# GuoYi0/alphaFive

Measured on AMD Instinct MI355X. Metric: self-play moves/sec (11x11, 500 sims/move), higher is better.
Workload: dtype f32 (fp16x2 split operands: 3 fp16 MFMA products per MAC, fp32 accumulate)

## Files before the change

alphafive_amd/csrc/af_engine.hip:

```cpp

#include <hip/hip_runtime.h>
#include <stdint.h>
#include <stdio.h>
#include <stdlib.h>
#include <string.h>

#include <type_traits>
#include <vector>

#include "af_engine.h"
#include "af_noise.h"

typedef unsigned long long u64;

enum { PH_IDLE = 0, PH_MOVE_START = 1, PH_SEARCH = 2, PH_MOVE_DONE = 3, PH_ERROR = 4, PH_DESCENT = 5  };
enum { CT_SIMS = 0, CT_SELECTS, CT_EXPANDS, CT_TERMINALS, CT_PLIES, CT_EPISODES, CT_LSUM, CT_LEXP,
       CT_GC, CT_GC_SCANNED, CT_YIELDS, CT_STALLS, CT_N };
enum { HIST_WORK = 0, HIST_TIME = 64, HIST_MAXTIME = 96, HIST_N = 97 };

struct EngineParams {
    int G, S, C, goal, sims, upper, training, mode, node_cap, max_ply, budget, budget_hard;
    uint32_t hash_mask;
    double init_temp, tau_decay, tau_decay_r, alpha, c_puct;
    float c_puct32;
// ... 191 lines not shown
            if (dir == 3) run_mask<KW, true>(theirs, d, P.goal, valid, wt);
            else run_mask<KW, false>(theirs, d, P.goal, valid, wt);
        } else if (dir == 3) {
            run_mask<KW, true>(mine, d, P.goal, valid, wm);
            run_mask<KW, true>(theirs, d, P.goal, valid, wt);
        } else {
            run_mask<KW, false>(mine, d, P.goal, valid, wm);
            run_mask<KW, false>(theirs, d, P.goal, valid, wt);
        }
#pragma unroll
        for (int k = 0; k < KW; ++k) any[k] = wm[k] | wt[k];
        const int f = bb_first<KW>(any);
        if (f >= 0) {
            const int key = f * 4 + dir;
            if (key < best_key) { best_key = key; best_v = bb_test<KW>(wm, f) ? 1.0f : -1.0f; }
        }
    }
    if (best_key != 0x7fffffff) { *value = best_v; return 1; }
    bool full = true;
#pragma unroll
    for (int k = 0; k < KW; ++k) full = full && ((mine[k] | theirs[k]) == P.boardmask[k]);
    *value = 0.0f;
    return full ? 1 : 0;
}

template <int KW>
__device__ __forceinline__ int terminal_through_last(const EngineParams& P, const u64* mine, const u64* theirs, int last, uint32_t inv_s16,
                                                     int lane, float* value) {
    const int S = P.S, g1 = P.goal - 1;
    const int y0 = (int)(((uint32_t)last * inv_s16) >> 16), x0 = last - y0 * S;
    const int dir = lane >> 4, j = (lane & 15) - g1;
    const int dy = dir == 1 ? 0 : (dir == 3 ? -1 : 1), dx = dir == 0 ? 0 : 1;
    const int y = y0 + j * dy, x = x0 + j * dx;
    const bool inb = (lane & 15) <= 2 * g1 && (unsigned)y < (unsigned)S && (unsigned)x < (unsigned)S;
    const int c = inb ? y * S + x : 0;
    u64 word = theirs[0];
#pragma unroll
    for (int k = 1; k < KW; ++k) word = (c >> 6) == k ? theirs[k] : word;
    const u64 w = __ballot(inb && ((word >> (c & 63)) & 1ull));
    u64 r = w;
    for (int t = 1; t <= g1; ++t) r &= w >> t;
    if (r) { *value = -1.0f; return 1; }
    bool full = true;
#pragma unroll
    for (int k = 0; k < KW; ++k) full = full && ((mine[k] | theirs[k]) == P.boardmask[k]);
    *value = 0.0f;
    return full ? 1 : 0;
}

template <int KW>
__host__ __device__ __forceinline__ uint32_t key_hash(const u64* mine, const u64* theirs) {
    u64 h = 0x9E3779B97F4A7C15ull;
#pragma unroll
    for (int k = 0; k < KW; ++k) {
        h = (h ^ mine[k]) * 0xff51afd7ed558ccdull;
        h ^= h >> 29;
        h = (h ^ theirs[k]) * 0xc4ceb9fe1a85ec53ull;
        h ^= h >> 32;
    }
    return (uint32_t)h;
}

template <int KW>
__device__ int tree_lookup(const EngineParams& P, int g, const u64* mine, const u64* theirs, int lane, uint32_t* slot_out) {
    const uint32_t* slots = P.hash + (size_t)g * (P.hash_mask + 1);
    const u64* keys = P.node_key + (size_t)g * P.node_cap * (2 * KW);
    const uint32_t h = key_hash<KW>(mine, theirs);
    for (uint32_t round = 0; round <= P.hash_mask / 64 + 1; ++round) {
        const uint32_t s = (h + round * 64 + lane) & P.hash_mask;
        const uint32_t v = slots[s];
        const u64 empties = __ballot(v == 0);
        const int first_empty = empties ? __builtin_ctzll(empties) : 64;
        bool match = false;
        if (v != 0 && lane < first_empty) {
            const u64* kk = keys + (size_t)(v - 1) * (2 * KW);
            match = true;
#pragma unroll
            for (int k = 0; k < KW; ++k) match = match && kk[k] == mine[k] && kk[KW + k] == theirs[k];
        }
        const u64 mm = __ballot(match);
        if (mm) {
            const int src = __builtin_ctzll(mm);
            return __builtin_amdgcn_readlane((int)v, src) - 1;
        }
        if (first_empty < 64) {
            *slot_out = (h + round * 64 + first_empty) & P.hash_mask;
            return -1;
        }
    }
    *slot_out = 0xffffffffu;
    return -1;
}

template <int KW>
__device__ __forceinline__ uint32_t memo_bucket(const EngineParams& P, const u64* mine, const u64* theirs, int last) {
    uint32_t h = key_hash<KW>(mine, theirs) ^ ((uint32_t)(last + 1) * 0x9E3779B1u);
    h ^= h >> 15; h *= 0x85EBCA6Bu; h ^= h >> 13;
    return h & P.memo_bucket_mask;
}
template <int KW>
__device__ __forceinline__ u64 memo_word(const EngineParams& P, const u64* mine, const u64* theirs, int last, int w) {
    const u64 kw = key_word<KW>(mine, theirs, w);
    return w == 2 * KW ? (((u64)P.memo_epoch << 32) | (u64)(uint32_t)(last + 1)) : kw;
}
template <int KW>
__device__ __forceinline__ int memo_probe(const EngineParams& P, uint32_t bucket, const u64* mine, const u64* theirs, int last, int lane,
                                          uint32_t* empty_ways) {
    constexpr int MK = 4 * KW;
    const int w = lane & (MK - 1);
    const u64 expect = memo_word<KW>(P, mine, theirs, last, w);
    u64 have = expect;
    if (lane < 4 * MK) have = P.memo_key[(size_t)bucket * (4 * MK) + lane];
    const u64 bad = __ballot(have != expect);
    const u64 blank = __ballot(lane < 4 * MK && w == 2 * KW && (uint32_t)(have >> 32) != P.memo_epoch);
    uint32_t em = 0;
    int hit = -1;
#pragma unroll
    for (int v = 3; v >= 0; --v) {
        const u64 wm = (MK == 16 ? 0xffffull : 0xffull) << (v * MK);
        if ((bad & wm) == 0ull) hit = (int)bucket * 4 + v;
        if (blank & wm) em |= 1u << v;
    }
    *empty_ways = em;
    return hit;
}


__device__ float pairwise_block(const float* a, int n) {
    if (n < 8) {
        float r = 0.0f;
        for (int i = 0; i < n; ++i) r = r + a[i];
        return r;
    }
    float r0 = a[0], r1 = a[1], r2 = a[2], r3 = a[3], r4 = a[4], r5 = a[5], r6 = a[6], r7 = a[7];
    int i;
    for (i = 8; i < n - (n % 8); i += 8) {
        r0 = r0 + a[i]; r1 = r1 + a[i + 1]; r2 = r2 + a[i + 2]; r3 = r3 + a[i + 3];
        r4 = r4 + a[i + 4]; r5 = r5 + a[i + 5]; r6 = r6 + a[i + 6]; r7 = r7 + a[i + 7];
    }
    float res = ((r0 + r1) + (r2 + r3)) + ((r4 + r5) + (r6 + r7));
    for (; i < n; ++i) res = res + a[i];
    return res;
}
__device__ float pairwise_sum(const float* a, int n) {
    if (n <= 128) return pairwise_block(a, n);
    int n2 = n / 2;
    n2 -= n2 % 8;
    return pairwise_block(a, n2) + pairwise_block(a + n2, n - n2);
}

#ifndef AF_TICK_MIN_WAVES
#define AF_TICK_MIN_WAVES 4
#endif
#ifdef AF_TICK_TIMING
__device__ unsigned long long g_tick_cycles[8192][13];
#define TK_T(var) const unsigned long long var = __builtin_readcyclecounter()
#define TK_ACC(slot, a, b) tk[slot] += (b) - (a)
#else
#define TK_T(var)
#define TK_ACC(slot, a, b)
#endif

template <int KW, bool W64, bool MEMO = false>
__global__ __launch_bounds__(64, AF_TICK_MIN_WAVES) void af_tick_kernel(EngineParams P, const float* __restrict__ policy_in,
                                                     const float* __restrict__ value_in, float* __restrict__ planes_out) {
    constexpr int CP = 64 * KW;
    __shared__ float s_pv[CP];
    __shared__ double s_cdf[CP];
    const int g = blockIdx.x;
    const int lane = threadIdx.x;
    const int C = P.C, NCAP = P.node_cap;
    if constexpr (MEMO) {
        if (g == 0 && lane == 0) atomicAdd(reinterpret_cast<unsigned long long*>(&P.memo_stats[MEMO_SERIAL]), 1ull);
    }

    int phase = rfli(P.phase[g]);
    if (phase == PH_IDLE || phase == PH_MOVE_DONE || phase == PH_ERROR) return;
    const u64 t_start = wall_clock64();
#ifdef AF_TICK_TIMING
    unsigned long long tk[13] = {0, 0, 0, 0, 0, 0, 0, 0, 0, 0, 0, 0, 0};
#endif
    TK_T(tk_entry);

    u64 root_m[KW], root_t[KW];
#pragma unroll
    for (int k = 0; k < KW; ++k) {
        root_m[k] = rfl64(P.root[(size_t)g * 2 * KW + k]);
        root_t[k] = rfl64(P.root[(size_t)g * 2 * KW + KW + k]);
    }
    int root_last = rfli(P.root_last[g]);
    int sims_left = rfli(P.sims_left[g]);
    int ply = rfli(P.ply[g]);
    int nodes = rfli(P.nodes[g]);
    int nfree = rfli(P.nfree[g]);
    double tau = P.tau[g];
    uint32_t episode = rfl32(P.episode[g]);
    uint32_t sel = rfl32(P.sel[g]);
    uint32_t plyctr = rfl32(P.plyctr[g]);
    const int random_a = rfli(P.random_a[g]);
    const uint32_t inv_s16 = (65536u + (uint32_t)P.S - 1u) / (uint32_t)P.S;
    const uint32_t k0 = P.k0, k1 = P.seed_hi + (P.first_game_id + (uint32_t)g);
    uint32_t ct[CT_N];
#pragma unroll
    for (int i = 0; i < CT_N; ++i) ct[i] = 0;
    int err = 0;

    u64* const nkeys = P.node_key + (size_t)g * NCAP * (2 * KW);
    int32_t* const nsum = P.node_sum + (size_t)g * NCAP;
    int32_t* const fre = P.free_idx + (size_t)g * NCAP;
    int32_t* const en = P.edge_n + (size_t)g * NCAP * CP;
    constexpr bool w64 = W64;
    float* const ew = P.edge_w + (w64 ? (size_t)0 : (size_t)g * NCAP * CP);
    double* const ew64 = P.edge_w64 + (w64 ? (size_t)g * NCAP * CP : (size_t)0);
    float* const ep = P.edge_p + (size_t)g * NCAP * CP;
    int32_t* const ec = P.edge_c + (size_t)g * NCAP * CP;
    uint32_t* const slots = P.hash + (size_t)g * (P.hash_mask + 1);
    int32_t* const pnode = P.path_node + (size_t)g * CP;
    int32_t* const pcell = P.path_cell + (size_t)g * CP;

    auto backup = [&](int depth, float v, int is_f32) {
        for (int d = lane; d < depth; d += 64) {
            const size_t off = (size_t)pnode[d] * CP + pcell[d];
            const float vv = ((depth - d) & 1) ? -v : v;
            const int32_t raw = en[off];
            if (w64) {
                en[off] = raw + 1;
                ew64[off] = ew64[off] + (double)vv;
            } else {
                en[off] = (raw + 1) | (is_f32 ? (int32_t)0x80000000 : 0);
                ew[off] = ew[off] + vv;
            }
        }
        __syncthreads();
    };

    TK_T(tk_loaded);
    TK_ACC(0, tk_entry, tk_loaded);
    u64 lm[KW], lt[KW];
    int c_depth = 0;
    uint32_t c_slot = 0;
    const float* c_pol = policy_in + (size_t)g * C;
    const float* c_val = value_in + g;
    bool have_eval = rfli(P.pending[g]) != 0;
    if (have_eval) {
#pragma unroll
        for (int k = 0; k < KW; ++k) {
            lm[k] = rfl64(P.leaf[(size_t)g * 2 * KW + k]);
            lt[k] = rfl64(P.leaf[(size_t)g * 2 * KW + KW + k]);
        }
        c_depth = rfli(P.depth[g]);
        c_slot = rfl32((uint32_t)P.leaf_slot[g]);
    }
    int status = AF_STATUS_IDLE;
    bool parked = false;
    int work = 0;
    uint32_t memo_probes = 0, memo_hits = 0;
  for (;;) {
    if (have_eval) {
        have_eval = false;
        u64 legal[KW];
#pragma unroll
        for (int k = 0; k < KW; ++k) legal[k] = ~(lm[k] | lt[k]) & P.boardmask[k];
        const int depth = c_depth;
        const uint32_t slot = c_slot;
        float pk[KW];
#pragma unroll
        for (int k = 0; k < KW; ++k) {
            const int c = lane + 64 * k;
            pk[k] = ((legal[k] >> lane) & 1ull) ? c_pol[c] : 0.0f;
        }
#pragma unroll
        for (int k = 0; k < KW; ++k) s_pv[lane + 64 * k] = pk[k];
        __syncthreads();
        float s = 0.0f;
#pragma unroll
        for (int i = 0; i < CP; i += 4) {
            const float4 v4 = *reinterpret_cast<const float4*>(&s_pv[i]);
            s = s + v4.x; s = s + v4.y; s = s + v4.z; s = s + v4.w;
        }
        s = rflf(s);
        if (!((double)s >= 1e-5)) s = (float)1e-5;
        if ((nfree == 0 && nodes >= NCAP) || slot == 0xffffffffu) {
            err = AF_ERR_NODE_CAP;
        } else {
            int idx;
            if (nfree > 0) idx = rfli(fre[--nfree]); else idx = nodes++;
            if (lane < 2 * KW) nkeys[(size_t)idx * 2 * KW + lane] = key_word<KW>(lm, lt, lane);
            if (lane == 0) {
                nsum[idx] = 0; slots[slot] = (uint32_t)idx + 1u;
                if (depth > 0) ec[(size_t)pnode[depth - 1] * CP + pcell[depth - 1]] = idx + 1;
            }
#pragma unroll
            for (int k = 0; k < KW; ++k) {
                const size_t off = (size_t)idx * CP + lane + 64 * k;
                en[off] = 0;
                ec[off] = 0;
                if (w64) ew64[off] = 0.0; else ew[off] = 0.0f;
                ep[off] = ((legal[k] >> lane) & 1ull) ? pk[k] / s : 0.0f;
            }
            __syncthreads();
            backup(depth, rflf(*c_val), 1);
            ct[CT_EXPANDS]++;
            ct[CT_LEXP] += (uint32_t)bb_count<KW>(legal);
        }
        ct[CT_SIMS]++;
        sims_left--;
    }

    TK_T(tk_consumed);
    TK_ACC(1, tk_loaded, tk_consumed);
    while (!parked && !err && !(MEMO && have_eval)) {
        TK_T(tk_iter);
        if (work >= ((MEMO && memo_hits) ? P.memo_budget : P.budget) && phase != PH_DESCENT) { status = AF_STATUS_YIELD; parked = true; ct[CT_YIELDS]++; break; }
        if (phase == PH_MOVE_START) {
            if (P.mode == AF_MODE_SELFPLAY && ply == 0 && rfl32(P.ep_seq[g]) - rfl32(P.ep_popped[g]) >= 2u) {
                status = AF_STATUS_YIELD; parked = true; ct[CT_STALLS]++;
                break;
            }
            bool collected = false;
            if (nodes - nfree + P.sims + 2 > NCAP && nodes > 0) {
                for (uint32_t s_ = lane; s_ <= P.hash_mask; s_ += 64) slots[s_] = 0;
                __syncthreads();
                const int rc = bb_count<KW>(root_m) + bb_count<KW>(root_t);
                int nf = 0;
                for (int base = 0; base < nodes; base += 64) {
                    const int i = base + lane;
                    const bool valid = i < nodes;
                    bool keep = false;
                    if (valid && nsum[i] >= 0) {
                        u64 nm[KW], nt[KW];
#pragma unroll
                        for (int k = 0; k < KW; ++k) { nm[k] = nkeys[(size_t)i * 2 * KW + k]; nt[k] = nkeys[(size_t)i * 2 * KW + KW + k]; }
                        const int nc = bb_count<KW>(nm) + bb_count<KW>(nt);
                        keep = true;
#pragma unroll
                        for (int k = 0; k < KW; ++k) {
                            const u64 a = ((nc ^ rc) & 1) ? nt[k] : nm[k];
                            const u64 b = ((nc ^ rc) & 1) ? nm[k] : nt[k];
                            keep = keep && ((a & root_m[k]) == root_m[k]) && ((b & root_t[k]) == root_t[k]);
                        }
                        if (keep) {
                            uint32_t h = key_hash<KW>(nm, nt);
                            for (;;) {
                                h &= P.hash_mask;
                                if (atomicCAS(&slots[h], 0u, (uint32_t)i + 1u) == 0u) break;
                                ++h;
                            }
                        } else {
                            nsum[i] = -1;
                        }
                    }
                    const u64 dm = __ballot(valid && !keep);
                    if (valid && !keep) fre[nf + __popcll(dm & ((1ull << lane) - 1ull))] = i;
                    nf += __popcll(dm);
                }
                nfree = nf;
                __syncthreads();
                __threadfence();
                ct[CT_GC]++; ct[CT_GC_SCANNED] += (uint32_t)nodes;
                collected = true;
            }
            uint32_t slot;
            const int ridx = tree_lookup<KW>(P, g, root_m, root_t, lane, &slot);
            int num = P.sims;
            if (ridx >= 0) { const int rem = P.upper - rfli(nsum[ridx]); num = rem < num ? rem : num; }
            sims_left = num;
            phase = PH_SEARCH;
            if (collected) { status = AF_STATUS_YIELD; parked = true; ct[CT_YIELDS]++; break; }
        }

        if (sims_left <= 0) {
            uint32_t slot;
            const int ridx = tree_lookup<KW>(P, g, root_m, root_t, lane, &slot);
            if (ridx < 0) { err = AF_ERR_NO_ROOT; break; }
            u64 legal[KW];
#pragma unroll
            for (int k = 0; k < KW; ++k) legal[k] = ~(root_m[k] | root_t[k]) & P.boardmask[k];
            const int L = bb_count<KW>(legal);
            int nv[KW];
            int most = -1;
#pragma unroll
            for (int k = 0; k < KW; ++k) {
                const bool lg = (legal[k] >> lane) & 1ull;
                nv[k] = lg ? (en[(size_t)ridx * CP + lane + 64 * k] & 0x7fffffff) : -1;
                most = nv[k] > most ? nv[k] : most;
            }
            most = wave_max_i32(most);
            u64 best[KW];
#pragma unroll
            for (int k = 0; k < KW; ++k) best[k] = __ballot(nv[k] == most && nv[k] >= 0);
            const int nb = bb_count<KW>(best);
            const uint32_t plyc = plyctr++;
            const int bi = (int)af_pick((uint32_t)nb, plyc, episode, AF_STREAM_BEST, k0, k1);
            const int best_cell = bb_select<KW>(best, bi);
            int action = best_cell, has_policy = 1;
            float pol[KW];
#pragma unroll
            for (int k = 0; k < KW; ++k) pol[k] = 0.0f;
            ct[CT_PLIES]++;
            if (lane == 0) atomicAdd(&P.progress[0], 1ull);
            if (!P.training && !random_a) {
                has_policy = 0;
            } else {
                tau = tau * (random_a ? P.tau_decay_r : P.tau_decay);
                if (tau <= 0.01) {
                    const float u = (float)(1.0 / (double)nb);
#pragma unroll
                    for (int k = 0; k < KW; ++k) pol[k] = ((best[k] >> lane) & 1ull) ? u : 0.0f;
                } else {
                    const float mx = (float)most;
                    const float inv_tau = (float)(1.0 / tau);
                    int e_idx[KW];
                    int base = 0;
#pragma unroll
                    for (int k = 0; k < KW; ++k) {
                        const bool lg = (legal[k] >> lane) & 1ull;
                        e_idx[k] = base + __popcll(legal[k] & ((1ull << lane) - 1ull));
                        base += __popcll(legal[k]);
                        if (lg) {
                            float x = (float)nv[k] / mx;
                            x = af_powf(x, inv_tau);
                            pol[k] = x;
                            s_pv[e_idx[k]] = x;
                        }
                    }
                    __syncthreads();
                    const float sum = pairwise_sum(s_pv, L);
                    __syncthreads();
#pragma unroll
                    for (int k = 0; k < KW; ++k) {
                        if ((legal[k] >> lane) & 1ull) { pol[k] = pol[k] / sum; s_pv[e_idx[k]] = pol[k]; }
                    }
                    __syncthreads();
                    if (lane == 0) {
                        double acc = 0.0;
                        for (int e = 0; e < L; ++e) { acc = acc + (double)s_pv[e]; s_cdf[e] = acc; }
                    }
                    __syncthreads();
                    const double last = s_cdf[L - 1];
                    const double u = af_uniform(plyc, episode, AF_STREAM_MOVE, k0, k1);
                    int cnt = 0;
#pragma unroll
                    for (int k = 0; k < KW; ++k) {
                        const bool lg = (legal[k] >> lane) & 1ull;
                        const bool le = lg && (s_cdf[e_idx[k]] / last <= u);
                        cnt += __popcll(__ballot(le));
                    }
                    __syncthreads();
                    if (cnt >= L) cnt = L - 1;
                    action = bb_select<KW>(legal, cnt);
                }
            }
#pragma unroll
            for (int k = 0; k < KW; ++k) {
                P.policy[(size_t)g * CP + lane + 64 * k] = pol[k];
                P.visits[(size_t)g * CP + lane + 64 * k] = nv[k] < 0 ? 0 : nv[k];
            }
            if (lane == 0) { P.action[g] = action; P.has_policy[g] = has_policy; }

            if (P.mode == AF_MODE_EXTERNAL) {
                phase = PH_MOVE_DONE;
                status = AF_STATUS_MOVE_DONE;
                parked = true;
                break;
            }
            if (ply >= P.max_ply) { err = AF_ERR_STATE; break; }
            const uint32_t seq = rfl32(P.ep_seq[g]);
            const size_t rslot = ((size_t)g * 2 + (seq & 1u)) * P.max_ply + ply;
            if (lane < 2 * KW) P.rec_key[rslot * 2 * KW + lane] = key_word<KW>(root_m, root_t, lane);
#pragma unroll
            for (int k = 0; k < KW; ++k) {
                const int c = lane + 64 * k;
                if (c < C) { P.rec_policy[rslot * C + c] = pol[k]; P.rec_visits[rslot * C + c] = nv[k] < 0 ? 0 : nv[k]; }
            }
            if (lane == 0) { P.rec_last[rslot] = root_last; P.rec_action[rslot] = action; }
            {
                u64 nm[KW], nt[KW];
#pragma unroll
                for (int k = 0; k < KW; ++k) { nm[k] = root_t[k]; nt[k] = root_m[k]; }
                bb_set<KW>(nt, action);
#pragma unroll
                for (int k = 0; k < KW; ++k) { root_m[k] = nm[k]; root_t[k] = nt[k]; }
            }
            root_last = action;
            ++ply;
            float fv;
            if (terminal_test<KW>(P, root_m, root_t, &fv)) {
                if (seq - rfl32(P.ep_popped[g]) >= 2u) { err = AF_ERR_EP_OVERRUN; break; }
                if (lane == 0) {
                    P.ep_len[(size_t)g * 2 + (seq & 1u)] = ply;
                    P.ep_final[(size_t)g * 2 + (seq & 1u)] = fv;
                    P.ep_seq[g] = seq + 1u;
                }
                ct[CT_EPISODES]++;
                if (lane == 0) atomicAdd(&P.progress[1], 1ull);
                for (uint32_t s_ = lane; s_ <= P.hash_mask; s_ += 64) slots[s_] = 0;
                __syncthreads();
                nodes = 0; nfree = 0;
#pragma unroll
                for (int k = 0; k < KW; ++k) { root_m[k] = 0; root_t[k] = 0; }
                root_last = -1;
                ply = 0;
                tau = P.init_temp;
                episode += 1; sel = 0; plyctr = 0;
            }
            phase = PH_MOVE_START;
            continue;
        }

        TK_T(tk_sim);
        TK_ACC(2, tk_iter, tk_sim);
        u64 cm[KW], ctb[KW];
        int last, depth;
        if (phase == PH_DESCENT) {
#pragma unroll
            for (int k = 0; k < KW; ++k) {
                cm[k] = rfl64(P.leaf[(size_t)g * 2 * KW + k]);
                ctb[k] = rfl64(P.leaf[(size_t)g * 2 * KW + KW + k]);
            }
            last = rfli(P.leaf_last[g]); depth = rfli(P.depth[g]);
            phase = PH_SEARCH;
        } else {
#pragma unroll
            for (int k = 0; k < KW; ++k) { cm[k] = root_m[k]; ctb[k] = root_t[k]; }
            last = root_last; depth = 0;
        }
        int hint = 0, pidx = -1, pcl = 0;
        typedef typename std::conditional<W64, double, float>::type wrow_t;
        int32_t r_raw[KW], r_c[KW];
        float r_p[KW];
        wrow_t r_w[KW];
        int32_t r_sum = 0;
        bool r_have = false;
        for (;;) {
            TK_T(tk_a);
            float tv;
            bool term;
            if (depth == 0)
                term = P.mode == AF_MODE_EXTERNAL ? (bool)terminal_test<KW, false>(P, cm, ctb, &tv) : false;
            else
                term = (depth > 0 && P.goal <= 8) ? (bool)terminal_through_last<KW>(P, cm, ctb, last, inv_s16, lane, &tv)
                                                                       : (bool)terminal_test<KW, true>(P, cm, ctb, &tv);
            if (term) {
                backup(depth, tv, 0);
                ct[CT_TERMINALS]++; ct[CT_SIMS]++;
                sims_left--;
                break;
            }
            uint32_t slot = 0xffffffffu;
            int idx;
            if (hint) {
                idx = hint - 1;
            } else {
                idx = tree_lookup<KW>(P, g, cm, ctb, lane, &slot);
                if (idx >= 0 && pidx >= 0 && lane == 0) ec[(size_t)pidx * CP + pcl] = idx + 1;
            }
            if (idx < 0) {
                if constexpr (MEMO) {
                    if (slot != 0xffffffffu && bb_count<KW>(cm) + bb_count<KW>(ctb) <= P.memo_max_stones) {
                        uint32_t unused;
                        const int me = memo_probe<KW>(P, memo_bucket<KW>(P, cm, ctb, last), cm, ctb, last, lane, &unused);
                        ++memo_probes;
                        if (me >= 0) {
                            ++memo_hits;
#pragma unroll
                            for (int k = 0; k < KW; ++k) { lm[k] = cm[k]; lt[k] = ctb[k]; }
                            c_depth = depth; c_slot = slot;
                            c_pol = P.memo_pv + (size_t)me * CP;
                            c_val = P.memo_val + me;
                            have_eval = true;
                            break;
                        }
                    }
                }
                if (lane < 2 * KW) P.leaf[(size_t)g * 2 * KW + lane] = key_word<KW>(cm, ctb, lane);
                if (lane == 0) { P.depth[g] = depth; P.leaf_last[g] = last; P.leaf_slot[g] = (int32_t)slot; }
                float* out = planes_out + (size_t)g * 3 * C;
#pragma unroll
                for (int k = 0; k < KW; ++k) {
                    const int c = lane + 64 * k;
                    if (c < C) {
                        out[c] = ((cm[k] >> lane) & 1ull) ? 1.0f : 0.0f;
                        out[C + c] = ((ctb[k] >> lane) & 1ull) ? 1.0f : 0.0f;
                        out[2 * C + c] = c == last ? 1.0f : 0.0f;
                    }
                }
                status = AF_STATUS_NEED_EVAL;
                parked = true;
                break;
            }
            if (work >= P.budget_hard) {
                if (lane < 2 * KW) P.leaf[(size_t)g * 2 * KW + lane] = key_word<KW>(cm, ctb, lane);
                if (lane == 0) { P.depth[g] = depth; P.leaf_last[g] = last; }
                phase = PH_DESCENT; status = AF_STATUS_YIELD; parked = true; ct[CT_YIELDS]++;
                break;
            }
            TK_T(tk_b);
            TK_ACC(3, tk_a, tk_b);
            const bool is_root = depth == 0;
            u64 legal[KW];
#pragma unroll
            for (int k = 0; k < KW; ++k) legal[k] = ~(cm[k] | ctb[k]) & P.boardmask[k];
            if (!r_have) {
                r_sum = nsum[idx];
#pragma unroll
                for (int k = 0; k < KW; ++k) {
                    const size_t off = (size_t)idx * CP + lane + 64 * k;
                    r_raw[k] = en[off];
                    r_c[k] = ec[off];
                    if constexpr (W64) r_w[k] = ew64[off]; else r_w[k] = ew[off];
                    r_p[k] = ep[off];
                }
            }
            r_have = false;
            const int sum_n = rfli(r_sum) + 1;
            if (lane == 0) nsum[idx] = sum_n;
            const uint32_t sel_id = sel++;
            int nn[KW];
            float pp[KW];
            wrow_t ww[KW];
            bool ff[KW];
            int32_t cc[KW];
#pragma unroll
            for (int k = 0; k < KW; ++k) {
                nn[k] = r_raw[k] & 0x7fffffff;
                ff[k] = r_raw[k] < 0;
                cc[k] = r_c[k];
                ww[k] = r_w[k];
                pp[k] = r_p[k];
            }
            double dd[KW];
            if (P.training) {
#ifdef AF_TICK_TIMING
                int tk_myit = 0;
#endif
                {
                    const float a_ = (float)P.alpha, inv_a = 1.0f / a_, one_m_a = 1.0f - a_;
                    uint32_t todo = 0;
#pragma unroll
                    for (int k = 0; k < KW; ++k) { dd[k] = 0.0; todo |= ((legal[k] >> lane) & 1ull) ? (1u << k) : 0u; }
                    af_u32x4 rk[KW];
                    uint32_t pend = 0;
#pragma unroll
                    for (int k = 0; k < KW; ++k) {
                        rk[k] = af_philox4x32(sel_id, episode, (AF_STREAM_GAMMA << 24) | (uint32_t)(lane + 64 * k), 0u, k0, k1);
                        float X;
                        const int ok = af_gamma_round(a_, inv_a, one_m_a, rk[k].v[0], rk[k].v[1], &X);
                        const bool lg = (todo >> k) & 1u;
                        dd[k] = (lg && ok) ? (double)X : 0.0;
                        pend |= (lg && !ok) ? (1u << k) : 0u;
                        if (KW > 2 && (k & 1)) __builtin_amdgcn_sched_barrier(0);
                    }
#ifdef AF_TICK_TIMING
                    ++tk_myit;
#endif
                    todo = pend;
                    {
                    uint32_t it = 1;
                    af_u32x4 r = rk[0];
#pragma unroll
                    for (int q = 1; q < KW; ++q) if (!(todo & ((1u << q) - 1u))) r = rk[q];
                    while (todo) {
#ifdef AF_TICK_TIMING
                        ++tk_myit;
#endif
                        const int k = __builtin_ctz(todo);
                        if ((it & 1u) == 0u) r = af_philox4x32(sel_id, episode, (AF_STREAM_GAMMA << 24) | (uint32_t)(lane + 64 * k), it >> 1, k0, k1);
                        const uint32_t wu = (it & 1u) ? r.v[2] : r.v[0], wv = (it & 1u) ? r.v[3] : r.v[1];
                        float X;
                        const int ok = af_gamma_round(a_, inv_a, one_m_a, wu, wv, &X);
                        if (ok || it == 0xFFFFu) {
                            const double Xd = ok ? (double)X : 0.0;
#pragma unroll
                            for (int q = 0; q < KW; ++q) dd[q] = q == k ? Xd : dd[q];
                            todo &= todo - 1u;
                            it = 1;
#pragma unroll
                            for (int q = 1; q < KW; ++q) if (todo && !(todo & ((1u << q) - 1u))) r = rk[q];
                        } else {
                            ++it;
                        }
                    }
                    }
                }
#ifdef AF_TICK_TIMING
                tk[12] += (unsigned long long)wave_max_i32(tk_myit);
#endif
                TK_T(tk_n1);
                TK_ACC(8, tk_b, tk_n1);
                double acc = 0.0;
#pragma unroll
                for (int k = 0; k < KW; ++k) acc = k == 0 ? dd[0] : acc + dd[k];
                acc = wave_sum_f64_tree(acc);
                if (acc == 0.0) {
                    int cnt = 0;
#pragma unroll
                    for (int k = 0; k < KW; ++k) cnt += __popcll(legal[k]);
                    const double u = 1.0 / (double)cnt;
#pragma unroll
                    for (int k = 0; k < KW; ++k) dd[k] = ((legal[k] >> lane) & 1ull) ? u : 0.0;
                } else {
                    const double inv = 1.0 / acc;
#pragma unroll
                    for (int k = 0; k < KW; ++k) dd[k] = dd[k] * inv;
                }
                TK_T(tk_n1e);
                TK_ACC(9, tk_n1, tk_n1e);
            }
            TK_T(tk_n2);
            const double sq = sqrt((double)(sum_n + 1));
            float sc[KW];
            float mx = -3.0e38f;
#pragma unroll
            for (int k = 0; k < KW; ++k) {
                const bool lg = (legal[k] >> lane) & 1ull;
                double q64;
                if (nn[k] == 0) q64 = 0.0;
                else if (!W64 && ff[k]) q64 = (double)((float)ww[k] / (float)nn[k]);
                else q64 = (double)ww[k] / (double)nn[k];
                double t;
                if (P.training) {
                    double p_;
                    if (is_root) p_ = (double)(0.75f * pp[k]) + 0.25 * dd[k];
                    else p_ = (double)(0.9f * pp[k]) + 0.1 * dd[k];
                    t = ((P.c_puct * p_) * sq) / (double)(1 + nn[k]);
                } else {
                    t = ((double)(P.c_puct32 * pp[k]) * sq) / (double)(1 + nn[k]);
                }
                sc[k] = lg ? (float)(q64 + t) : -3.0e38f;
                mx = sc[k] > mx ? sc[k] : mx;
            }
            TK_T(tk_n3);
            TK_ACC(10, tk_n2, tk_n3);
            int cell = -1;
            if (is_root && P.training) {
                u64 cand[KW];
#pragma unroll
                for (int k = 0; k < KW; ++k) cand[k] = __ballot(((legal[k] >> lane) & 1ull) && nn[k] == 0);
                int m = bb_count<KW>(cand);
                if (m == 0) {
#pragma unroll
                    for (int k = 0; k < KW; ++k) cand[k] = __ballot(((legal[k] >> lane) & 1ull) && nn[k] == 1);
                    m = bb_count<KW>(cand);
                }
                if (m > 0) cell = bb_select_wave<KW>(cand, (int)af_pick((uint32_t)m, sel_id, episode, AF_STREAM_PICK, k0, k1), lane);
            }
            if (cell < 0) {
                mx = wave_max_f32(mx);
                u64 cand[KW];
#pragma unroll
                for (int k = 0; k < KW; ++k) cand[k] = __ballot(((legal[k] >> lane) & 1ull) && sc[k] == mx);
                const int m = bb_count<KW>(cand);
                cell = bb_select_wave<KW>(cand, (int)af_pick((uint32_t)m, sel_id, episode, AF_STREAM_PICK, k0, k1), lane);
            }
            cell = rfli(cell);
            hint = 0;
#pragma unroll
            for (int k = 0; k < KW; ++k) { const int t_ = __builtin_amdgcn_readlane(cc[k], cell & 63); if ((cell >> 6) == k) hint = t_; }
            hint = rfli(hint);
            pidx = idx; pcl = cell;
            if (hint) {
                const int ci = hint - 1;
                r_sum = nsum[ci];
#pragma unroll
                for (int k = 0; k < KW; ++k) {
                    const size_t off = (size_t)ci * CP + lane + 64 * k;
                    r_raw[k] = en[off];
                    r_c[k] = ec[off];
                    if constexpr (W64) r_w[k] = ew64[off]; else r_w[k] = ew[off];
                    r_p[k] = ep[off];
                }
                r_have = true;
            }
            ++work;
            ct[CT_SELECTS]++;
            ct[CT_LSUM] += (uint32_t)bb_count<KW>(legal);
            if (lane == 0) { pnode[depth] = idx; pcell[depth] = cell; }
            ++depth;
            {
                u64 nm[KW], nt[KW];
#pragma unroll
                for (int k = 0; k < KW; ++k) { nm[k] = ctb[k]; nt[k] = cm[k]; }
                bb_set<KW>(nt, cell);
#pragma unroll
                for (int k = 0; k < KW; ++k) { cm[k] = nm[k]; ctb[k] = nt[k]; }
            }
            last = cell;
            __syncthreads();
            TK_T(tk_c);
            TK_ACC(4, tk_b, tk_c);
            TK_ACC(11, tk_n3, tk_c);
#ifdef AF_TICK_TIMING
            tk[7] += 1;
#endif
        }
    }
    if (!MEMO || !have_eval) break;
  }
    TK_T(tk_parked);
    if constexpr (MEMO) {
        if (lane == 0 && memo_probes) {
            atomicAdd(reinterpret_cast<unsigned long long*>(&P.memo_stats[MEMO_PROBES]), (unsigned long long)memo_probes);
            if (memo_hits) atomicAdd(reinterpret_cast<unsigned long long*>(&P.memo_stats[MEMO_HITS]), (unsigned long long)memo_hits);
        }
    }

    if (err) { phase = PH_ERROR; status = err; }
    if (lane < 2 * KW) P.root[(size_t)g * 2 * KW + lane] = key_word<KW>(root_m, root_t, lane);
    if (lane == 0) {
        P.phase[g] = phase;
        P.pending[g] = status == AF_STATUS_NEED_EVAL ? 1 : 0;
        P.root_last[g] = root_last;
        P.sims_left[g] = sims_left;
        P.ply[g] = ply;
        P.nodes[g] = nodes;
        P.nfree[g] = nfree;
        P.tau[g] = tau;
        P.episode[g] = episode;
        P.sel[g] = sel;
        P.plyctr[g] = plyctr;
        P.status[g] = status;
        for (int i = 0; i < CT_N; ++i)
            if (ct[i]) atomicAdd(reinterpret_cast<unsigned long long*>(&P.counters[(size_t)g * CT_N + i]), (unsigned long long)ct[i]);
        const u64 dt = wall_clock64() - t_start;
        atomicAdd(&P.hist[HIST_WORK + (work < 63 ? work : 63)], 1ull);
        const u64 tb = dt / 800ull;
        atomicAdd(&P.hist[HIST_TIME + (tb < 31ull ? tb : 31ull)], 1ull);
        atomicMax(&P.hist[HIST_MAXTIME], dt);
    }
#ifdef AF_TICK_TIMING
    {
        TK_T(tk_end);
        tk[5] = tk_end - tk_parked;
        tk[6] = tk_end - tk_entry;
        if (lane == 0 && g < 8192) for (int q = 0; q < 13; ++q) g_tick_cycles[g][q] = tk[q];
    }
#endif
}

__global__ __launch_bounds__(1024) void af_pack_scan(EngineParams P, int max_eps, int max_plies, int32_t* __restrict__ out) {
    __shared__ int s_e[1024], s_p[1024];
    __shared__ int s_cut;
    const int t = threadIdx.x;
    int base_e = 0, base_p = 0;
    int32_t* meta = out + 4;
    int32_t* fin = out + 4 + (size_t)max_eps * 4;
    if (t == 0) s_cut = 0x7fffffff;
    __syncthreads();
    for (int g0 = 0; g0 < P.G; g0 += 1024) {
        const int g = g0 + t;
        int ne = 0, T0 = 0, T1 = 0;
        uint32_t pop = 0;
        if (g < P.G) {
            pop = P.ep_popped[g];
            ne = (int)(P.ep_seq[g] - pop);
            if (ne >= 1) T0 = P.ep_len[(size_t)g * 2 + (pop & 1u)];
            if (ne >= 2) T1 = P.ep_len[(size_t)g * 2 + ((pop + 1u) & 1u)];
        }
        s_e[t] = ne; s_p[t] = T0 + T1;
        __syncthreads();
        for (int off = 1; off < 1024; off <<= 1) {
            const int ve = t >= off ? s_e[t - off] : 0, vp = t >= off ? s_p[t - off] : 0;
            __syncthreads();
            s_e[t] += ve; s_p[t] += vp;
            __syncthreads();
        }
        const int e_excl = base_e + s_e[t] - ne, p_excl = base_p + s_p[t] - (T0 + T1);
        int fit = 0;
        if (ne >= 1 && e_excl + 1 <= max_eps && p_excl + T0 <= max_plies) {
            fit = 1;
            if (ne >= 2 && e_excl + 2 <= max_eps && p_excl + T0 + T1 <= max_plies) fit = 2;
        }
        if (g < P.G && fit < ne) atomicMin(&s_cut, g);
        __syncthreads();
        const int cut = s_cut;
        if (g < P.G && g <= cut && fit > 0) {
            for (int k = 0; k < fit; ++k) {
                const uint32_t seq = pop + (uint32_t)k;
                const int idx = e_excl + k;
                meta[idx * 4 + 0] = g; meta[idx * 4 + 1] = (int32_t)seq;
                meta[idx * 4 + 2] = k == 0 ? T0 : T1; meta[idx * 4 + 3] = p_excl + (k == 0 ? 0 : T0);
                fin[idx] = __float_as_int(P.ep_final[(size_t)g * 2 + (seq & 1u)]);
            }
            P.ep_popped[g] = pop + (uint32_t)fit;
        }
        __syncthreads();
        if (cut != 0x7fffffff) {
            if (g == cut) {
                out[0] = e_excl + fit;
                out[1] = p_excl + (fit >= 1 ? T0 : 0) + (fit >= 2 ? T1 : 0);
            }
            break;
        }
        base_e += s_e[1023]; base_p += s_p[1023];
        __syncthreads();
    }
    __syncthreads();
    if (t == 0) {
        if (s_cut == 0x7fffffff) { out[0] = base_e; out[1] = base_p; }
        out[2] = 2 * (P.C <= 128 ? 2 : 4); out[3] = P.C;
    }
}

__global__ __launch_bounds__(256) void af_pack_copy(EngineParams P, int max_eps, int32_t* __restrict__ out) {
    const int idx = blockIdx.x;
    if (idx >= out[0]) return;
    const int32_t* meta = out + 4 + (size_t)idx * 4;
    const int g = meta[0], T = meta[2], poff = meta[3];
    const uint32_t seq = (uint32_t)meta[1];
    const int C = P.C, KW2 = 2 * (C <= 128 ? 2 : 4), R = 2 * KW2 + 2 * C + 2;
    const size_t r0 = ((size_t)g * 2 + (seq & 1u)) * P.max_ply;
    int32_t* dst = out + 4 + (size_t)max_eps * 5 + (size_t)poff * R;
    const int32_t* keys = reinterpret_cast<const int32_t*>(P.rec_key + r0 * KW2);
    const int32_t* pol = reinterpret_cast<const int32_t*>(P.rec_policy + r0 * C);
    const int32_t* vis = P.rec_visits + r0 * C;
    for (int i = threadIdx.x; i < T * R; i += blockDim.x) {
        const int ply = i / R, f = i - ply * R;
        int32_t v;
        if (f < 2 * KW2) v = keys[(size_t)ply * 2 * KW2 + f];
        else if (f < 2 * KW2 + C) v = pol[(size_t)ply * C + (f - 2 * KW2)];
        else if (f < 2 * KW2 + 2 * C) v = vis[(size_t)ply * C + (f - 2 * KW2 - C)];
        else if (f == 2 * KW2 + 2 * C) v = P.rec_last[r0 + ply];
        else v = P.rec_action[r0 + ply];
        dst[i] = v;
    }
}

__device__ __forceinline__ void install_root(const EngineParams& P, int g, int lane, int KW2, u64 word, int last, int ra, int reset) {
    if (reset) {
        uint32_t* slots = P.hash + (size_t)g * (P.hash_mask + 1);
        for (uint32_t s_ = lane; s_ <= P.hash_mask; s_ += 64) slots[s_] = 0;
        if (lane == 0) { P.nodes[g] = 0; P.nfree[g] = 0; P.tau[g] = P.init_temp; P.episode[g] += 1; P.sel[g] = 0; P.plyctr[g] = 0; }
    }
    if (lane < KW2) P.root[(size_t)g * KW2 + lane] = word;
    if (lane == 0) { P.root_last[g] = last; P.random_a[g] = ra ? 1 : 0; P.phase[g] = PH_MOVE_START; P.pending[g] = 0; P.status[g] = 0; }
}

__global__ __launch_bounds__(64) void af_set_roots_kernel(EngineParams P, int n, const int32_t* __restrict__ req, const u64* __restrict__ keys, int KW2) {
    const int i = blockIdx.x, lane = threadIdx.x;
    if (i >= n) return;
    const int g = req[4 * i], last = req[4 * i + 1], ra = req[4 * i + 2], reset = req[4 * i + 3];
    install_root(P, g, lane, KW2, lane < KW2 ? keys[(size_t)i * KW2 + lane] : 0ull, last, ra, reset);
}

// ... 890 lines not shown
```

Baseline: 6083.

## Batch Dirichlet gamma draws ahead into shared ring and compact rejection retries

Result: no change. 6072 (-0.2%).

```diff
diff --git a/alphafive_amd/csrc/af_engine.hip b/alphafive_amd/csrc/af_engine.hip
--- a/alphafive_amd/csrc/af_engine.hip
+++ b/alphafive_amd/csrc/af_engine.hip
@@ -367,6 +367,9 @@
 #ifndef AF_TICK_MIN_WAVES
 #define AF_TICK_MIN_WAVES 4
 #endif
+#ifndef AF_TICK_AHEAD_FROM
+#define AF_TICK_AHEAD_FROM 1
+#endif
 #ifdef AF_TICK_TIMING
 __device__ unsigned long long g_tick_cycles[8192][13];
 #define TK_T(var) const unsigned long long var = __builtin_readcyclecounter()
@@ -382,6 +385,9 @@
     constexpr int CP = 64 * KW;
     __shared__ float s_pv[CP];
     __shared__ double s_cdf[CP];
+    constexpr int RJ = 8 / KW;
+    __shared__ uint2 s_ring[RJ * CP];
+    __shared__ uint16_t s_work[RJ * CP];
     const int g = blockIdx.x;
     const int lane = threadIdx.x;
     const int C = P.C, NCAP = P.node_cap;
@@ -447,6 +453,66 @@
             }
         }
         __syncthreads();
+    };
+
+    uint32_t ring_from = 0, ring_n = 0;
+    auto draw = [&](uint32_t sel_from, uint32_t n, const u64 (&mask)[KW]) {
+        const float a_ = (float)P.alpha, inv_a = 1.0f / a_, one_m_a = 1.0f - a_;
+        uint32_t pend = 0;
+#ifdef AF_TICK_TIMING
+        int tk_myit = 0;
+#endif
+        for (uint32_t j = 0; j < n; ++j) {
+#pragma unroll
+            for (int k = 0; k < KW; ++k) {
+                const af_u32x4 r = af_philox4x32(sel_from + j, episode, (AF_STREAM_GAMMA << 24) | (uint32_t)(lane + 64 * k), 0u, k0, k1);
+                float X;
+                const int ok = af_gamma_round(a_, inv_a, one_m_a, r.v[0], r.v[1], &X);
+                const bool rej = ((mask[k] >> lane) & 1ull) && !ok;
+                s_ring[j * CP + lane + 64 * k] = rej ? make_uint2(r.v[2], r.v[3]) : make_uint2(ok ? __float_as_uint(X) : 0u, 0u);
+                pend |= rej ? (1u << (j * KW + k)) : 0u;
+                if (KW > 2 && (k & 1)) __builtin_amdgcn_sched_barrier(0);
+            }
+#ifdef AF_TICK_TIMING
+            ++tk_myit;
+#endif
+        }
+        uint32_t total = 0;
+        for (uint32_t b = 0; b < n * KW; ++b) {
+            const bool mine = (pend >> b) & 1u;
+            const u64 m = __ballot(mine);
+            if (mine) s_work[total + __builtin_amdgcn_mbcnt_hi((uint32_t)(m >> 32), __builtin_amdgcn_mbcnt_lo((uint32_t)m, 0u))] =
+                (uint16_t)((b / KW) * CP + lane + 64 * (b % KW));
+            total += (uint32_t)__popcll(m);
+        }
+        __syncthreads();
+        for (uint32_t base = 0; base < total; base += 64) {
+            bool live = base + lane < total;
+            const uint32_t idx = live ? s_work[base + lane] : 0u;
+            const uint2 w = s_ring[idx];
+            const uint32_t wsel = sel_from + idx / CP, wcell = (AF_STREAM_GAMMA << 24) | (idx % CP);
+            uint32_t it = 1;
+            af_u32x4 r = {{0u, 0u, w.x, w.y}};
+            while (live) {
+#ifdef AF_TICK_TIMING
+                ++tk_myit;
+#endif
+                if ((it & 1u) == 0u) r = af_philox4x32(wsel, episode, wcell, it >> 1, k0, k1);
+                const uint32_t wu = (it & 1u) ? r.v[2] : r.v[0], wv = (it & 1u) ? r.v[3] : r.v[1];
+                float X;
+                const int ok = af_gamma_round(a_, inv_a, one_m_a, wu, wv, &X);
+                if (ok || it == 0xFFFFu) {
+                    s_ring[idx].x = ok ? __float_as_uint(X) : 0u;
+                    live = false;
+                } else {
+                    ++it;
+                }
+            }
+        }
+        __syncthreads();
+#ifdef AF_TICK_TIMING
+        tk[12] += (unsigned long long)wave_max_i32(tk_myit);
+#endif
     };
 
     TK_T(tk_loaded);
@@ -718,6 +784,7 @@
                 ply = 0;
                 tau = P.init_temp;
                 episode += 1; sel = 0; plyctr = 0;
+                ring_n = 0;
             }
             phase = PH_MOVE_START;
             continue;
@@ -844,109 +911,6 @@
                 ww[k] = r_w[k];
                 pp[k] = r_p[k];
             }
-            double dd[KW];
-            if (P.training) {
-#ifdef AF_TICK_TIMING
-                int tk_myit = 0;
-#endif
-                {
-                    const float a_ = (float)P.alpha, inv_a = 1.0f / a_, one_m_a = 1.0f - a_;
-                    uint32_t todo = 0;
-#pragma unroll
-                    for (int k = 0; k < KW; ++k) { dd[k] = 0.0; todo |= ((legal[k] >> lane) & 1ull) ? (1u << k) : 0u; }
-                    af_u32x4 rk[KW];
-                    uint32_t pend = 0;
-#pragma unroll
-                    for (int k = 0; k < KW; ++k) {
-                        rk[k] = af_philox4x32(sel_id, episode, (AF_STREAM_GAMMA << 24) | (uint32_t)(lane + 64 * k), 0u, k0, k1);
-                        float X;
-                        const int ok = af_gamma_round(a_, inv_a, one_m_a, rk[k].v[0], rk[k].v[1], &X);
-                        const bool lg = (todo >> k) & 1u;
-                        dd[k] = (lg && ok) ? (double)X : 0.0;
-                        pend |= (lg && !ok) ? (1u << k) : 0u;
-                        if (KW > 2 && (k & 1)) __builtin_amdgcn_sched_barrier(0);
-                    }
-#ifdef AF_TICK_TIMING
-                    ++tk_myit;
-#endif
-                    todo = pend;
-                    {
-                    uint32_t it = 1;
-                    af_u32x4 r = rk[0];
-#pragma unroll
-                    for (int q = 1; q < KW; ++q) if (!(todo & ((1u << q) - 1u))) r = rk[q];
-                    while (todo) {
-#ifdef AF_TICK_TIMING
-                        ++tk_myit;
-#endif
-                        const int k = __builtin_ctz(todo);
-                        if ((it & 1u) == 0u) r = af_philox4x32(sel_id, episode, (AF_STREAM_GAMMA << 24) | (uint32_t)(lane + 64 * k), it >> 1, k0, k1);
-                        const uint32_t wu = (it & 1u) ? r.v[2] : r.v[0], wv = (it & 1u) ? r.v[3] : r.v[1];
-                        float X;
-                        const int ok = af_gamma_round(a_, inv_a, one_m_a, wu, wv, &X);
-                        if (ok || it == 0xFFFFu) {
-                            const double Xd = ok ? (double)X : 0.0;
-#pragma unroll
-                            for (int q = 0; q < KW; ++q) dd[q] = q == k ? Xd : dd[q];
-                            todo &= todo - 1u;
-                            it = 1;
-#pragma unroll
-                            for (int q = 1; q < KW; ++q) if (todo && !(todo & ((1u << q) - 1u))) r = rk[q];
-                        } else {
-                            ++it;
-                        }
-                    }
-                    }
-                }
-#ifdef AF_TICK_TIMING
-                tk[12] += (unsigned long long)wave_max_i32(tk_myit);
-#endif
-                TK_T(tk_n1);
-                TK_ACC(8, tk_b, tk_n1);
-                double acc = 0.0;
-#pragma unroll
-                for (int k = 0; k < KW; ++k) acc = k == 0 ? dd[0] : acc + dd[k];
-                acc = wave_sum_f64_tree(acc);
-                if (acc == 0.0) {
-                    int cnt = 0;
-#pragma unroll
-                    for (int k = 0; k < KW; ++k) cnt += __popcll(legal[k]);
-                    const double u = 1.0 / (double)cnt;
-#pragma unroll
-                    for (int k = 0; k < KW; ++k) dd[k] = ((legal[k] >> lane) & 1ull) ? u : 0.0;
-                } else {
-                    const double inv = 1.0 / acc;
-#pragma unroll
-                    for (int k = 0; k < KW; ++k) dd[k] = dd[k] * inv;
-                }
-                TK_T(tk_n1e);
-                TK_ACC(9, tk_n1, tk_n1e);
-            }
-            TK_T(tk_n2);
-            const double sq = sqrt((double)(sum_n + 1));
-            float sc[KW];
-            float mx = -3.0e38f;
-#pragma unroll
-            for (int k = 0; k < KW; ++k) {
-                const bool lg = (legal[k] >> lane) & 1ull;
-                double q64;
-                if (nn[k] == 0) q64 = 0.0;
-                else if (!W64 && ff[k]) q64 = (double)((float)ww[k] / (float)nn[k]);
-                else q64 = (double)ww[k] / (double)nn[k];
-                double t;
-                if (P.training) {
-                    double p_;
-                    if (is_root) p_ = (double)(0.75f * pp[k]) + 0.25 * dd[k];
-                    else p_ = (double)(0.9f * pp[k]) + 0.1 * dd[k];
-                    t = ((P.c_puct * p_) * sq) / (double)(1 + nn[k]);
-                } else {
-                    t = ((double)(P.c_puct32 * pp[k]) * sq) / (double)(1 + nn[k]);
-                }
-                sc[k] = lg ? (float)(q64 + t) : -3.0e38f;
-                mx = sc[k] > mx ? sc[k] : mx;
-            }
-            TK_T(tk_n3);
-            TK_ACC(10, tk_n2, tk_n3);
             int cell = -1;
             if (is_root && P.training) {
                 u64 cand[KW];
@@ -960,13 +924,89 @@
                 }
                 if (m > 0) cell = bb_select_wave<KW>(cand, (int)af_pick((uint32_t)m, sel_id, episode, AF_STREAM_PICK, k0, k1), lane);
             }
+#ifdef AF_TICK_TIMING
+            unsigned long long tk_scored = __builtin_readcyclecounter();
+            tk[8] += tk_scored - tk_b;
+#endif
             if (cell < 0) {
-                mx = wave_max_f32(mx);
-                u64 cand[KW];
-#pragma unroll
-                for (int k = 0; k < KW; ++k) cand[k] = __ballot(((legal[k] >> lane) & 1ull) && sc[k] == mx);
-                const int m = bb_count<KW>(cand);
-                cell = bb_select_wave<KW>(cand, (int)af_pick((uint32_t)m, sel_id, episode, AF_STREAM_PICK, k0, k1), lane);
+                double dd[KW];
+                if (P.training) {
+                    uint32_t rj = sel_id - ring_from;
+                    if (rj >= ring_n) {
+                        uint32_t n = 1;
+                        if (work >= AF_TICK_AHEAD_FROM) {
+                            const int cap = (work < P.budget && P.budget < P.budget_hard) ? P.budget : P.budget_hard;
+                            n = (uint32_t)(cap - work);
+                            n = n < (uint32_t)RJ ? n : (uint32_t)RJ;
+                        }
+                        u64 dmask[KW];
+#pragma unroll
+                        for (int k = 0; k < KW; ++k) dmask[k] = n == 1 ? legal[k] : (~(root_m[k] | root_t[k]) & P.boardmask[k]);
+                        draw(sel_id, n, dmask);
+                        ring_from = sel_id; ring_n = n; rj = 0;
+                    }
+#pragma unroll
+                    for (int k = 0; k < KW; ++k) {
+                        const float X = __uint_as_float(s_ring[rj * CP + lane + 64 * k].x);
+                        dd[k] = ((legal[k] >> lane) & 1ull) ? (double)X : 0.0;
+                    }
+                    TK_T(tk_n1);
+                    TK_ACC(8, tk_scored, tk_n1);
+                    double acc = 0.0;
+#pragma unroll
+                    for (int k = 0; k < KW; ++k) acc = k == 0 ? dd[0] : acc + dd[k];
+                    acc = wave_sum_f64_tree(acc);
+                    if (acc == 0.0) {
+                        int cnt = 0;
+#pragma unroll
+                        for (int k = 0; k < KW; ++k) cnt += __popcll(legal[k]);
+                        const double u = 1.0 / (double)cnt;
+#pragma unroll
+                        for (int k = 0; k < KW; ++k) dd[k] = ((legal[k] >> lane) & 1ull) ? u : 0.0;
+                    } else {
+                        const double inv = 1.0 / acc;
+#pragma unroll
+                        for (int k = 0; k < KW; ++k) dd[k] = dd[k] * inv;
+                    }
+                    TK_T(tk_n1e);
+                    TK_ACC(9, tk_n1, tk_n1e);
+                }
+                TK_T(tk_n2);
+                const double sq = sqrt((double)(sum_n + 1));
+                float sc[KW];
+                float mx = -3.0e38f;
+#pragma unroll
+                for (int k = 0; k < KW; ++k) {
+                    const bool lg = (legal[k] >> lane) & 1ull;
+                    double q64;
+                    if (nn[k] == 0) q64 = 0.0;
+                    else if (!W64 && ff[k]) q64 = (double)((float)ww[k] / (float)nn[k]);
+                    else q64 = (double)ww[k] / (double)nn[k];
+                    double t;
+                    if (P.training) {
+                        double p_;
+                        if (is_root) p_ = (double)(0.75f * pp[k]) + 0.25 * dd[k];
+                        else p_ = (double)(0.9f * pp[k]) + 0.1 * dd[k];
+                        t = ((P.c_puct * p_) * sq) / (double)(1 + nn[k]);
+                    } else {
+                        t = ((double)(P.c_puct32 * pp[k]) * sq) / (double)(1 + nn[k]);
+                    }
+                    sc[k] = lg ? (float)(q64 + t) : -3.0e38f;
+                    mx = sc[k] > mx ? sc[k] : mx;
+                }
+                TK_T(tk_n3);
+                TK_ACC(10, tk_n2, tk_n3);
+#ifdef AF_TICK_TIMING
+                tk_scored = tk_n3;
+#endif
+                {
+                    mx = wave_max_f32(mx);
+                    u64 cand[KW];
+#pragma unroll
+                    for (int k = 0; k < KW; ++k) cand[k] = __ballot(((legal[k] >> lane) & 1ull) && sc[k] == mx);
+                    const int m = bb_count<KW>(cand);
+                    cell = bb_select_wave<KW>(cand, (int)af_pick((uint32_t)m, sel_id, episode, AF_STREAM_PICK, k0, k1), lane);
+                }
             }
             cell = rfli(cell);
             hint = 0;
@@ -1004,7 +1044,9 @@
             __syncthreads();
             TK_T(tk_c);
             TK_ACC(4, tk_b, tk_c);
-            TK_ACC(11, tk_n3, tk_c);
+#ifdef AF_TICK_TIMING
+            tk[11] += tk_c - tk_scored;
+#endif
 #ifdef AF_TICK_TIMING
             tk[7] += 1;
 #endif
```
